# lh3/miniasm

Measured on NVIDIA H100. Metric: paf_overlaps_per_sec_ingest_to_gfa, higher is better.
Workload: dtype int64/uint32 (+3 float32 predicates)

## Files before the change

### miniasm_b200/csrc/asg_dev.cu

```cuda
#include "asg_dev.cuh"
#include <cub/cub.cuh>

int mab_verbose = 3;
thread_local int mab_mute = 0;
int mab_del_trans_count_inner = 0;
thread_local DelTransStats g_del_trans_stats;

__device__ __forceinline__ DArc ld_arc(const DArc *p)
{
	uint4 t = *reinterpret_cast<const uint4*>(p);
	DArc a;
	a.ul = (uint64_t)t.y << 32 | t.x; a.v = t.z; a.ol_del = t.w;
	return a;
}
__device__ __forceinline__ DArc ld_arc_nc(const DArc *p)
{
	uint4 t = __ldg(reinterpret_cast<const uint4*>(p));
	DArc a;
	a.ul = (uint64_t)t.y << 32 | t.x; a.v = t.z; a.ol_del = t.w;
	return a;
}

__device__ __forceinline__ uint4 ld_arc4(const DArc *p)
{
// ... 47 lines not shown
	{
		DArc a = ld_arc_nc(arc + i);
		if (flag && flag[i]) return false;
		if (a.ol_del & MAB_DEL_BIT) return false;
		uint32_t u = (uint32_t)(a.ul >> 32);
		return !((seq[u >> 1] | seq[a.v >> 1]) & MAB_DEL_BIT);
	}
};

__global__ void k_arc_count_dead(ArcKeep keep, uint32_t n, unsigned long long *n_dead)
{
	unsigned dead = 0;
	for (uint32_t i = blockIdx.x * blockDim.x + threadIdx.x; i < n; i += gridDim.x * blockDim.x) dead += !keep(i);
	dead = __reduce_add_sync(0xffffffffu, dead);
	if ((threadIdx.x & 31) == 0 && dead) atomicAdd(n_dead, (unsigned long long)dead);
}

void dg_arc_rm(MabDev &d, DGraph &g, const uint8_t *flag)
{
	if (g.n_arc == 0) return;
	cub::CountingInputIterator<uint32_t> cnt(0);
	ArcKeep keep{g.arc, g.seq, flag};
	if (!flag && g.n_arc > (1u << 20)) {
		d.zero_scal(SC_NSEL);
		MAB_LAUNCH(d, k_arc_count_dead, mab_grid(g.n_arc, 256), 256, 0, keep, g.n_arc, d.d_scal + SC_NSEL);
		if (d.get_scal(SC_NSEL) == 0) return;
	}
	cub::TransformInputIterator<bool, ArcKeep, cub::CountingInputIterator<uint32_t>> flags(cnt, keep);
	size_t tb = 0;
	unsigned long long *d_n = d.d_scal + SC_NSEL;
// ... 606 lines not shown
```

### miniasm_b200/csrc/asg_dev.cuh

```cuda
#pragma once
#include "mab_common.cuh"

struct DGraph {
	uint32_t n_seq = 0;
	uint32_t n_arc = 0;
	size_t   m_arc = 0;
	bool is_srt = false, is_symm = false, has_idx = false;
	uint32_t len_bits = 32;
	DArc *arc = nullptr;
	DArc *arc2 = nullptr;
	uint32_t *seq = nullptr;
	uint64_t *idx = nullptr;
};

void dg_reserve(MabDev &d, DGraph &g, size_t m_arc);
void dg_set_nseq(MabDev &d, DGraph &g, uint32_t n_seq);
void dg_free(MabDev &d, DGraph &g);

void dg_arc_rm(MabDev &d, DGraph &g, const uint8_t *flag);
void dg_arc_sort(MabDev &d, DGraph &g);
void dg_build_sorted(MabDev &d, DGraph &g, uint64_t *key, uint64_t *val, uint64_t *key2, uint64_t *val2, uint32_t n_in, uint32_t n_real, uint32_t lb, bool has_sentinel);
void dg_arc_index(MabDev &d, DGraph &g);
void dg_cleanup(MabDev &d, DGraph &g, const uint8_t *flag = nullptr);
uint32_t dg_del_multi(MabDev &d, DGraph &g);
uint32_t dg_del_asymm(MabDev &d, DGraph &g);
void dg_symm(MabDev &d, DGraph &g);
uint32_t dg_del_trans(MabDev &d, DGraph &g, uint32_t fuzz);
uint32_t dg_del_trans_flags(MabDev &d, DGraph &g, uint32_t fuzz, uint32_t own_lo, uint32_t own_hi, uint8_t **flag_out,
                            const DArc *const *peer = nullptr, const uint64_t *nidx = nullptr, const uint32_t *orig = nullptr, uint32_t world = 1);
uint32_t dg_del_short(MabDev &d, DGraph &g, float ratio);

struct DelTransStats { uint64_t n_arc_in, n_vtx, inner_iters, n_reduced, n_big; float kernel_ms; };
extern thread_local DelTransStats g_del_trans_stats;

// ... 5 lines not shown
```

### miniasm_b200/csrc/capi_fused.cu

```cuda
#include "../../include/miniasm_b200.h"
#include "capi_util.cuh"
#include "hit_dev.cuh"
#include "clean_dev.cuh"
#include "gfa_dev.cuh"
#include "dump_dev.cuh"
#include "ugseq_dev.cuh"
#include <pthread.h>
#include "ingest_dev.cuh"
#include "shard_comm.cuh"
#include <cub/cub.cuh>
#include <map>
#include <string>
#include <zlib.h>
#include <fcntl.h>
#include <unistd.h>
#include <sys/stat.h>

ma_ug_t *mab_ug_download(MabDev &d, DUnitigs &du);
extern "C" sdict_t *sd_from_packed(char *block, size_t block_size, uint32_t n, const uint32_t *len);

struct mab_ctx {
	MabDev dev;
	char *d_text = nullptr;
	size_t text_len = 0, text_cap = 0;
// ... 793 lines not shown
	dg_arc_rm(d, loc, nullptr);
	DGraph &g = c->sg;
	uint32_t n_keep = 0;
	DArc *keep = nullptr;
	uint64_t n_red_all = 0, tot = 0;
	std::vector<uint64_t> cnt = sc_allgather_u64(d, sc, loc.n_arc);
	for (int r = 0; r < G; ++r) tot += cnt[r];
	if (tot >= (1ull << 31)) { fprintf(stderr, "[E::miniasm_b200] more than 2^31 arcs in the graph\n"); exit(73); }
	c->stats.n_arc_sg = tot;
	if (MAB_V(1)) fprintf(stderr, "[M::%s] read %d arcs\n", "ma_sg_gen", (int)tot);
	std::vector<void*> peer_any;
	const bool p2p = sc_peer_ptrs(d, sc, loc.arc, peer_any);
	std::vector<const DArc*> peer_ptr((size_t)G, nullptr);
	for (int r = 0; r < G; ++r) peer_ptr[r] = (const DArc*)peer_any[r];
	if (p2p) {
		dg_arc_index(d, loc);
		uint64_t *nidx = mab_alloc<uint64_t>(d, (size_t)n * 2);
		if (n) MAB_CUDA(cudaMemcpyAsync(nidx, loc.idx, (size_t)n * 16, cudaMemcpyDeviceToDevice, d.stream));
		sc_allreduce(d, sc, nidx, (size_t)n * 2, ncclUint64, ncclSum);
		const DArc **d_peer = (const DArc**)d.alloc(sizeof(void*) * (size_t)G);
		MAB_CUDA(cudaMemcpyAsync(d_peer, peer_ptr.data(), sizeof(void*) * (size_t)G, cudaMemcpyHostToDevice, d.stream));
		uint8_t *flag = nullptr;
		uint32_t n_red = dg_del_trans_flags(d, loc, (uint32_t)opt->gap_fuzz, 0, 0xffffffffu, &flag, d_peer, nidx, c->orig_id, (uint32_t)G);
		c->stats.ms_del_trans_kernel = g_del_trans_stats.kernel_ms, c->stats.trans_inner = g_del_trans_stats.inner_iters;
		std::vector<uint64_t> reds = sc_allgather_u64(d, sc, n_red);
		for (int r = 0; r < G; ++r) n_red_all += reds[r];
		keep = mab_alloc<DArc>(d, loc.n_arc);
		if (loc.n_arc) {
			uint8_t *nf = mab_alloc<uint8_t>(d, loc.n_arc);
			MAB_LAUNCH(d, k_not_flag, mab_grid(loc.n_arc, 256), 256, 0, flag, loc.n_arc, nf);
			size_t tb = 0;
// ... 68 lines not shown
```

### miniasm_b200/csrc/hit_dev.cu

```cuda
#include "hit_dev.cuh"
#include "hit2arc.cuh"
#include <cub/cub.cuh>
#include <functional>

extern "C" int ma_verbose;
extern "C" const char *sys_timestamp(void);
#define ma_verbose_dev (mab_mute ? 0 : ma_verbose)

thread_local MabCountHook mab_count_hook = nullptr;
thread_local void *mab_count_hook_ctx = nullptr;
static inline void sum_ranks(unsigned long long *v, int n) { if (mab_count_hook) mab_count_hook(mab_count_hook_ctx, v, n); }

__device__ __forceinline__ DHit ld_hit(const DHit *p)
{
	const uint4 *q = reinterpret_cast<const uint4*>(p);
	uint4 a = __ldg(q), b = __ldg(q + 1);
	DHit h;
	h.qns = (uint64_t)a.y << 32 | a.x; h.qe = a.z; h.tn = a.w;
	h.ts = b.x; h.te = b.y; h.ml_rev = b.z; h.bl_del = b.w;
	return h;
}
__device__ __forceinline__ DHit ld_hit_rw(const DHit *p)
{
	const uint4 *q = reinterpret_cast<const uint4*>(p);
// ... 385 lines not shown
{
	drop_bounds(d, h);
	const uint32_t n_seq = h.n_seq;
	if (h.n == 0 || n_seq == 0) return;
	if (h.n >= (1ull << 32)) { fprintf(stderr, "[E::miniasm_b200] more than 2^32 hits on one GPU\n"); exit(73); }
	uint32_t *cnt = mab_alloc<uint32_t>(d, (size_t)n_seq + 1), *first = mab_alloc<uint32_t>(d, (size_t)n_seq + 1);
	MAB_CUDA(cudaMemsetAsync(cnt, 0, ((size_t)n_seq + 1) * 4, d.stream));
	MAB_LAUNCH(d, k_bucket_count, mab_grid(h.n, 256), 256, 0, h.a, h.n, cnt);
	dh_bucket_first(d, cnt, n_seq, first);
	MAB_CUDA(cudaMemsetAsync(cnt, 0, (size_t)n_seq * 4, d.stream));
	MAB_LAUNCH(d, k_bucket_fill, mab_grid(h.n, 256), 256, 0, h.a, h.n, first, cnt, h.a2);
	dh_sort_buckets(d, h, first);
	d.free(cnt); d.free(first);
}

__global__ void k_group_bounds(const DHit *a, size_t n, uint32_t *g32)
{
	for (size_t i = blockIdx.x * (size_t)blockDim.x + threadIdx.x; i < n; i += (size_t)gridDim.x * blockDim.x) {
		uint32_t q = (uint32_t)(a[i].qns >> 32);
		if (i == 0 || (uint32_t)(a[i - 1].qns >> 32) != q) g32[2 * (size_t)q + 1] = (uint32_t)i;
		if (i == n - 1 || (uint32_t)(a[i + 1].qns >> 32) != q) g32[2 * (size_t)q] = (uint32_t)(i + 1);
	}
}

__global__ void k_sub_keys(const DHit *a, size_t n, const uint64_t *__restrict__ grp, float min_iden, uint32_t clip, uint64_t *key)
{
	for (size_t i = blockIdx.x * (size_t)blockDim.x + threadIdx.x; i < n; i += (size_t)gridDim.x * blockDim.x) {
		DHit h = ld_hit(a + i);
		uint32_t qid = (uint32_t)(h.qns >> 32);
		int ml = (int)(h.ml_rev & 0x7fffffffu), bl = (int)(h.bl_del & 0x7fffffffu);
		bool skip = i >= (uint32_t)grp[qid] || h.tn == qid || (float)ml < __fmul_rn((float)bl, min_iden);
		uint32_t qs = (uint32_t)h.qns + clip, qe = h.qe - clip;
		uint64_t base = (uint64_t)qid << 33;
		if (!skip && qe > qs) {
			key[2 * i] = base | (uint32_t)(qs << 1);
			key[2 * i + 1] = base | (uint32_t)(qe << 1 | 1);
		} else {
// ... 339 lines not shown
	}
	d.free(huge);
}

uint64_t dh_sub(MabDev &d, const DHits &h, int min_dp, float min_iden, int end_clip, DSub *sub_out)
{
	const uint32_t n_seq = h.n_seq;
	unsigned long long n_remained = 0;
	if (n_seq) MAB_CUDA(cudaMemsetAsync(sub_out, 0, (size_t)n_seq * sizeof(DSub), d.stream));
	if (h.n && n_seq) {
		if (h.n >= (1ull << 31)) { fprintf(stderr, "[E::miniasm_b200] more than 2^31 hits on one GPU\n"); exit(73); }
		uint64_t *grp = h.grp;
		if (!grp) {
			grp = mab_alloc<uint64_t>(d, n_seq);
			MAB_CUDA(cudaMemsetAsync(grp, 0, (size_t)n_seq * 8, d.stream));
			MAB_LAUNCH(d, k_group_bounds, mab_grid(h.n, 256), 256, 0, h.a, h.n, (uint32_t*)grp);
		}
		uint32_t *big = mab_alloc<uint32_t>(d, n_seq);
		MAB_CUDA(cudaMemsetAsync(d.d_scal, 0, 8 * sizeof(unsigned long long), d.stream));
		unsigned grid = (n_seq + SUBW_WARPS - 1) / SUBW_WARPS;
		if (grid > MAB_SMS * 32u) grid = MAB_SMS * 32u;
		MAB_LAUNCH(d, k_sub_warp, grid, SUBW_WARPS * 32, 0, h.a, grp, n_seq, min_dp, min_iden, (uint32_t)end_clip, sub_out, big, d.d_scal);
		uint32_t n_big = (uint32_t)d.get_scal(SC_BIG);
		if (n_big) sub_big_reads(d, h, grp, big, n_big, min_dp, min_iden, end_clip, sub_out);
		n_remained = d.get_scal(SC_COUNT);
		if (grp != h.grp) d.free(grp);
		d.free(big);
	}
	sum_ranks(&n_remained, 1);
	if (ma_verbose_dev >= 3)
		fprintf(stderr, "[M::%s::%s] %ld query sequences remain after sub\n", "ma_hit_sub", sys_timestamp(), (long)n_remained);
// ... 327 lines not shown
	const int lane = threadIdx.x & 31;
	for (uint32_t r = (blockIdx.x * blockDim.x + threadIdx.x) >> 5; r < n_seq; r += (gridDim.x * blockDim.x) >> 5) {
		const int32_t m = map[r];
		if (m < 0) continue;
		const uint64_t g = grp[r];
		const uint32_t end = (uint32_t)g, first = (uint32_t)(g >> 32);
		unsigned c = 0;
		if (end) for (uint32_t i = first + lane; i < end; i += 32) c += map[tn[i]] >= 0;
		c = __reduce_add_sync(0xffffffffu, c);
		if (lane == 0) cnt[m] = c;
	}
}

__global__ void __launch_bounds__(256)
k_sel_final_copy(const DHit *__restrict__ a, const uint64_t *__restrict__ grp, const int32_t *__restrict__ map, uint32_t n_seq,
                 const uint32_t *__restrict__ off, const uint32_t *__restrict__ n_new, DHit *__restrict__ out, unsigned long long *scal)
{
	const int lane = threadIdx.x & 31;
	const unsigned lt = (1u << lane) - 1u;
	if (blockIdx.x == 0 && threadIdx.x == 0) { const uint32_t nn = *n_new; scal[SCS_NSEQ] = nn, scal[SCS_NHITS] = off[nn]; }
	for (uint32_t r = (blockIdx.x * blockDim.x + threadIdx.x) >> 5; r < n_seq; r += (gridDim.x * blockDim.x) >> 5) {
		const int32_t m = map[r];
		if (m < 0) continue;
		const uint64_t g = grp[r];
		const uint32_t end = (uint32_t)g, first = (uint32_t)(g >> 32);
		if (end == 0) continue;
		uint32_t o = off[m];
		for (uint32_t c = first; c < end; c += 32) {
			const uint32_t i = c + lane;
			DHit h;
			int32_t tn = -1;
			if (i < end) { h = ld_hit(a + i); tn = map[h.tn]; }
			const unsigned km = __ballot_sync(0xffffffffu, tn >= 0);
			if (tn >= 0) {
				h.qns = (uint64_t)(uint32_t)m << 32 | (uint32_t)h.qns, h.tn = (uint32_t)tn;
				st_hit(out + o + __popc(km & lt), h);
			}
			o += __popc(km);
// ... 11 lines not shown
{
	size_t tb = 0;
	cub::DeviceScan::ExclusiveSum(nullptr, tb, in, out, (int64_t)n, d.stream);
	void *tmp = d.tmp(tb);
	cub::DeviceScan::ExclusiveSum(tmp, tb, in, out, (int64_t)n, d.stream);
	++d.n_lib;
}

size_t dh_select(MabDev &d, DHits &h, DSub *sub, const SelectParams &o, int32_t *map_out, float *cov, const SelectHooks &hk)
{
	const uint32_t n_seq = h.n_seq;
	if (h.n >= (1ull << 31)) { fprintf(stderr, "[E::miniasm_b200] more than 2^31 hits on one GPU\n"); exit(73); }
	if (!h.grp) {
		h.grp = mab_alloc<uint64_t>(d, n_seq);
		MAB_CUDA(cudaMemsetAsync(h.grp, 0, (size_t)n_seq * 8, d.stream));
		if (h.n) MAB_LAUNCH(d, k_group_bounds, mab_grid(h.n, 256), 256, 0, h.a, h.n, (uint32_t*)h.grp);
	}
	dh_sub(d, h, o.min_dp, o.min_iden, 0, sub);
	if (hk.sub_done) hk.sub_done(sub);
	d.trace("select:sub1");

	const int clip = o.min_span / 2;
	DSub *sub2 = mab_alloc<DSub>(d, n_seq);
	uint32_t *big = mab_alloc<uint32_t>(d, n_seq);
	MAB_CUDA(cudaMemsetAsync(sub2, 0, (size_t)n_seq * sizeof(DSub), d.stream));
	d.zero_scal(0, SCS_NHITS + 1);
	MAB_LAUNCH(d, k_sel_cut_flt_sub, warp_grid(n_seq, SUBW_WARPS), SUBW_WARPS * 32, 0, h.a, h.grp, n_seq, sub, o.min_span, o.flt_max_hang, o.flt_min_ovlp,
	           o.min_dp, o.min_iden, (uint32_t)clip, sub2, big, d.d_scal);
	const uint32_t n_big = (uint32_t)d.get_scal(SC_BIG);
	{
		unsigned long long gv[4] = { d.h_scal[SCS_DP], d.h_scal[SCS_LEN], d.h_scal[SCS_CUT], d.h_scal[SCS_FLT] };
// ... 18 lines not shown

	uint8_t *used = mab_alloc<uint8_t>(d, n_seq);
	uint32_t *tn = reinterpret_cast<uint32_t*>(h.a2);
	MAB_CUDA(cudaMemsetAsync(used, 0, n_seq, d.stream));
	MAB_LAUNCH(d, k_sel_cut_cont, warp_grid(n_seq, 8), 256, 0, h.a, h.grp, n_seq, sub2, sub, o.min_span, o.cont, used, tn, d.d_scal + SCS_CUT2);
	if (hk.flags_done) hk.flags_done(sub, used, n_seq);

	uint32_t *keep = mab_alloc<uint32_t>(d, (size_t)n_seq + 1), *excl = mab_alloc<uint32_t>(d, (size_t)n_seq + 1);
	uint32_t *cnt = mab_alloc<uint32_t>(d, (size_t)n_seq + 1), *off = mab_alloc<uint32_t>(d, (size_t)n_seq + 1);
	MAB_CUDA(cudaMemsetAsync(keep + n_seq, 0, 4, d.stream));
	MAB_LAUNCH(d, k_cont_keep, mab_grid(n_seq, 256), 256, 0, n_seq, sub, used, nullptr, keep);
	exclusive_sum(d, keep, excl, (size_t)n_seq + 1);
	MAB_LAUNCH(d, k_cont_map, mab_grid(n_seq, 256), 256, 0, n_seq, keep, excl, map_out, sub, sub2);
	MAB_LAUNCH(d, k_sel_final_count, warp_grid(n_seq, 8), 256, 0, h.grp, tn, map_out, n_seq, cnt);
	exclusive_sum(d, cnt, off, (size_t)n_seq + 1);
	MAB_LAUNCH(d, k_sel_final_copy, warp_grid(n_seq, 8), 256, 0, h.a, h.grp, map_out, n_seq, off, excl + n_seq, h.a2, d.d_scal);
	const uint32_t n_new = (uint32_t)d.get_scal(SCS_NSEQ);
	const size_t n_hits = (size_t)d.h_scal[SCS_NHITS];
	const unsigned long long n_cut2 = d.h_scal[SCS_CUT2];
	if (n_new) MAB_CUDA(cudaMemcpyAsync(sub, sub2, (size_t)n_new * sizeof(DSub), cudaMemcpyDeviceToDevice, d.stream));
	d.free(sub2); d.free(used); d.free(keep); d.free(excl); d.free(cnt); d.free(off);
	DHit *t = h.a; h.a = h.a2; h.a2 = t;
	h.n = n_hits, h.n_seq = n_new;
	drop_bounds(d, h);
	d.trace("select:cut2+contained");

	unsigned long long gv[2] = { n_cut2, (unsigned long long)h.n };
	sum_ranks(gv, 2);
	if (ma_verbose_dev >= 3) {
		fprintf(stderr, "[M::%s::%s] %ld hits remain after cut\n", "ma_hit_cut", sys_timestamp(), (long)gv[0]);
		fprintf(stderr, "[M::%s::%s] %d sequences and %ld hits remain after containment removal\n", "ma_hit_contained", sys_timestamp(), n_new, (long)gv[1]);
	}
	return h.n;
}

__global__ void k_seq_set(uint32_t n_seq, const uint32_t *len, const uint8_t *del, uint32_t *seq, unsigned *max_len)
{
	unsigned mx = 0;
	for (uint32_t i = blockIdx.x * blockDim.x + threadIdx.x; i < n_seq; i += gridDim.x * blockDim.x) {
// ... 17 lines not shown
		bool emit = false;
		if (r >= 0) {
			if (qn == h.tn) {
				if ((uint32_t)h.qns == h.ts && h.qe == h.te && (h.ml_rev >> 31)) atomicOr(&seq[qn], MAB_DEL_BIT);
			} else emit = true;
		} else if (r == MAB_HT_QCONT) atomicOr(&seq[qn], MAB_DEL_BIT);
		key[i] = emit ? ((t.ul >> 32) << lb | (uint32_t)t.ul) : sentinel;
		val[i] = (uint64_t)t.ol_del << 32 | t.v;
		cnt += emit;
	}
	cnt = __reduce_add_sync(0xffffffffu, cnt);
	if ((threadIdx.x & 31) == 0 && cnt) atomicAdd(n_emit, (unsigned long long)cnt);
}

constexpr int SGW_WARPS = 8, SGW_HITS = 256, SGW_IDX_BITS = 9;
constexpr int SGC_HITS = 8192;

__global__ void k_sg_classify(const DHit *a, size_t n, uint32_t *seq, HitArcParams p, uint8_t *emit_flag, uint32_t *g32, unsigned long long *scal)
{
	unsigned cnt = 0;
	bool bad = false;
	for (size_t i = blockIdx.x * (size_t)blockDim.x + threadIdx.x; i < n; i += (size_t)gridDim.x * blockDim.x) {
		DHit h = ld_hit(a + i);
		const uint32_t qn = (uint32_t)(h.qns >> 32);
		DArc t;
		t.ul = 0, t.v = 0, t.ol_del = 0;
		const int r = mab_hit2arc(h, (int)(seq[qn] & 0x7fffffffu), (int)(seq[h.tn] & 0x7fffffffu), p.max_hang, p.int_frac, p.min_ovlp, &t);
		bool emit = false;
		if (r >= 0) {
			if (qn == h.tn) {
				if ((uint32_t)h.qns == h.ts && h.qe == h.te && (h.ml_rev >> 31)) atomicOr(&seq[qn], MAB_DEL_BIT);
			} else emit = true;
		} else if (r == MAB_HT_QCONT) atomicOr(&seq[qn], MAB_DEL_BIT);
		emit_flag[i] = emit;
		cnt += emit;
		const uint32_t prev = i ? (uint32_t)(a[i - 1].qns >> 32) : 0;
		if (i == 0 || prev != qn) g32[2 * (size_t)qn + 1] = (uint32_t)i;
		if (i == n - 1 || (uint32_t)(a[i + 1].qns >> 32) != qn) g32[2 * (size_t)qn] = (uint32_t)(i + 1);
		if (i && prev > qn) bad = true;
	}
	cnt = __reduce_add_sync(0xffffffffu, cnt);
	if ((threadIdx.x & 31) == 0 && cnt) atomicAdd(scal + SC_COUNT, (unsigned long long)cnt);
	if (bad) scal[SC_AUX2] = 1ull;
}

struct U8ToU32 { __host__ __device__ __forceinline__ uint32_t operator()(uint8_t x) const { return x; } };

__global__ void __launch_bounds__(SGW_WARPS * 32)
k_sg_sort_warp(const DHit *__restrict__ a, const uint64_t *__restrict__ grp, const uint32_t *__restrict__ epos, const uint32_t *__restrict__ seq,
               uint32_t n_seq, HitArcParams p, uint32_t lb, DArc *__restrict__ out, uint32_t *big_list, unsigned long long *scal)
{
	__shared__ uint32_t s_key[SGW_WARPS][SGW_HITS], s_v[SGW_WARPS][SGW_HITS], s_ol[SGW_WARPS][SGW_HITS];
	const int warp = threadIdx.x >> 5, lane = threadIdx.x & 31;
	uint32_t *key = s_key[warp], *pv = s_v[warp], *pol = s_ol[warp];
	const uint32_t len_mask = (1u << lb) - 1u;
	for (uint32_t r = blockIdx.x * SGW_WARPS + warp; r < n_seq; r += gridDim.x * SGW_WARPS) {
		const uint64_t g = grp[r];
		const uint32_t end = (uint32_t)g, first = (uint32_t)(g >> 32);
		if (end == 0) continue;
		const uint32_t cnt = end - first;
		if (cnt > SGW_HITS) { if (lane == 0) big_list[atomicAdd(scal + SC_BIG, 1ull)] = r; continue; }
		const int ql = (int)(seq[r] & 0x7fffffffu);
		uint32_t n = 0;
		for (uint32_t c = 0; c < cnt; c += 32) {
			bool ok = false;
			DArc t;
			t.ul = 0, t.v = 0, t.ol_del = 0;
			if (c + lane < cnt) {
				const DHit h = ld_hit(a + first + c + lane);
				const int rr = mab_hit2arc(h, ql, (int)(seq[h.tn] & 0x7fffffffu), p.max_hang, p.int_frac, p.min_ovlp, &t);
				ok = rr >= 0 && h.tn != r;
			}
			const unsigned m = __ballot_sync(0xffffffffu, ok);
			if (ok) {
				const uint32_t k = n + __popc(m & ((1u << lane) - 1u));
				key[k] = ((((uint32_t)(t.ul >> 32) & 1u) << lb | (uint32_t)t.ul) << SGW_IDX_BITS) | k;
				pv[k] = t.v, pol[k] = t.ol_del;
			}
			n += __popc(m);
		}
		if (n == 0) continue;
		uint32_t np = 32; while (np < n) np <<= 1;
		__syncwarp();
		switch (np) {
			case 32: sub_sort_regs<1>(key, n, lane); break;
			case 64: sub_sort_regs<2>(key, n, lane); break;
			case 128: sub_sort_regs<4>(key, n, lane); break;
			default: sub_sort_regs<8>(key, n, lane); break;
		}
		__syncwarp();
		const uint32_t base = epos[first];
		for (uint32_t j = lane; j < n; j += 32) {
			const uint32_t k = key[j], src = k & ((1u << SGW_IDX_BITS) - 1u), kl = k >> SGW_IDX_BITS;
			*reinterpret_cast<uint4*>(out + base + j) = make_uint4(kl & len_mask, r << 1 | kl >> lb, pv[src], pol[src]);
		}
		__syncwarp();
	}
}

__global__ void __launch_bounds__(512)
k_sg_sort_cta(const DHit *__restrict__ a, const uint64_t *__restrict__ grp, const uint32_t *__restrict__ epos, const uint32_t *__restrict__ seq,
              const uint32_t *__restrict__ big_list, uint32_t n_big, HitArcParams p, DArc *__restrict__ out, unsigned long long *scal)
{
	extern __shared__ __align__(16) unsigned char sg_smem[];
	uint64_t *key = reinterpret_cast<uint64_t*>(sg_smem);
	uint32_t *pv = reinterpret_cast<uint32_t*>(key + SGC_HITS), *pol = pv + SGC_HITS;
	__shared__ uint32_t s_n;
	const uint32_t tid = threadIdx.x, nt = blockDim.x;
	for (uint32_t b = blockIdx.x; b < n_big; b += gridDim.x) {
		const uint32_t r = big_list[b];
		const uint64_t g = grp[r];
		const uint32_t first = (uint32_t)(g >> 32), cnt = (uint32_t)g - first;
		if (cnt > SGC_HITS) { if (tid == 0) atomicAdd(scal + SC_AUX, 1ull); continue; }
		if (tid == 0) s_n = 0;
		__syncthreads();
		const uint32_t base = epos[first];
		const int ql = (int)(seq[r] & 0x7fffffffu);
		for (uint32_t c = tid; c < cnt; c += nt) {
			const DHit h = ld_hit(a + first + c);
			DArc t;
			t.ul = 0, t.v = 0, t.ol_del = 0;
			const int rr = mab_hit2arc(h, ql, (int)(seq[h.tn] & 0x7fffffffu), p.max_hang, p.int_frac, p.min_ovlp, &t);
			if (rr >= 0 && h.tn != r) {
				const uint32_t k = epos[first + c] - base;
				key[k] = (uint64_t)((((uint32_t)(t.ul >> 32) & 1u) << 31) | (uint32_t)t.ul) << 32 | k;
				pv[k] = t.v, pol[k] = t.ol_del;
				atomicAdd(&s_n, 1u);
			}
		}
		__syncthreads();
		const uint32_t n = s_n;
		uint32_t np = 2; while (np < n) np <<= 1;
		for (uint32_t i = n + tid; i < np; i += nt) key[i] = ~0ull;
		__syncthreads();
		for (uint32_t k = 2, lk = 1; k <= np; k <<= 1, ++lk)
			for (uint32_t lj = lk; lj-- > 0;) {
				const uint32_t j = 1u << lj;
				for (uint32_t t = tid; t < np / 2; t += nt) {
					const uint32_t lo = ((t >> lj) << (lj + 1)) | (t & (j - 1)), hi = lo + j;
					const uint64_t x = key[lo], y = key[hi];
					const bool asc = (lo & k) == 0;
					if ((x > y) == asc) key[lo] = y, key[hi] = x;
				}
				__syncthreads();
			}
		for (uint32_t j = tid; j < n; j += nt) {
			const uint64_t k = key[j];
			const uint32_t src = (uint32_t)k, kl = (uint32_t)(k >> 32);
			*reinterpret_cast<uint4*>(out + base + j) = make_uint4(kl & 0x7fffffffu, r << 1 | kl >> 31, pv[src], pol[src]);
		}
		__syncthreads();
	}
}

static bool sg_emit_segmented(MabDev &d, const DHits &h, const HitArcParams &p, uint32_t lb, DGraph &g)
{
	const size_t n = h.n;
	const uint32_t n_seq = h.n_seq;
	if (lb + 1 + SGW_IDX_BITS > 32 || n >= (1ull << 31)) return false;
	uint8_t *ef = mab_alloc<uint8_t>(d, n);
	uint32_t *epos = mab_alloc<uint32_t>(d, n), *big = mab_alloc<uint32_t>(d, n_seq);
	uint64_t *grp = mab_alloc<uint64_t>(d, n_seq);
	MAB_CUDA(cudaMemsetAsync(grp, 0, (size_t)n_seq * 8, d.stream));
	d.zero_scal(SC_COUNT, 5);
	MAB_LAUNCH(d, k_sg_classify, mab_grid(n, 256), 256, 0, h.a, n, g.seq, p, ef, (uint32_t*)grp, d.d_scal);
	const uint32_t n_arc = (uint32_t)d.get_scal(SC_COUNT);
	bool ok = d.h_scal[SC_AUX2] == 0;
	if (ok) {
		cub::TransformInputIterator<uint32_t, U8ToU32, const uint8_t*> in(ef, U8ToU32());
		size_t tb = 0;
		cub::DeviceScan::ExclusiveSum(nullptr, tb, in, epos, (int64_t)n, d.stream);
		void *tmp = d.tmp(tb);
		cub::DeviceScan::ExclusiveSum(tmp, tb, in, epos, (int64_t)n, d.stream);
		++d.n_lib;
		dg_reserve(d, g, n_arc ? n_arc : 1);
		unsigned grid = (n_seq + SGW_WARPS - 1) / SGW_WARPS;
		if (grid > MAB_SMS * 32u) grid = MAB_SMS * 32u;
		MAB_LAUNCH(d, k_sg_sort_warp, grid, SGW_WARPS * 32, 0, h.a, grp, epos, g.seq, n_seq, p, lb, g.arc, big, d.d_scal);
		const uint32_t n_big = (uint32_t)d.get_scal(SC_BIG);
		if (n_big) {
				const size_t smem = (size_t)SGC_HITS * 16;
			MAB_CUDA(cudaFuncSetAttribute(k_sg_sort_cta, cudaFuncAttributeMaxDynamicSharedMemorySize, (int)smem));
			MAB_LAUNCH(d, k_sg_sort_cta, n_big < MAB_SMS ? n_big : MAB_SMS, 512, smem, h.a, grp, epos, g.seq, big, n_big, p, g.arc, d.d_scal);
			if (d.get_scal(SC_AUX) != 0) ok = false;
		}
	}
	d.free(ef); d.free(epos); d.free(big); d.free(grp);
	if (ok) g.len_bits = lb, g.n_arc = n_arc, g.is_srt = true, g.has_idx = false;
	return ok;
}

void dh_sg_gen(MabDev &d, const DHits &h, const uint32_t *len, const uint8_t *del, const HitArcParams &p, DGraph &g)
{
	dh_sg_emit(d, h, len, del, p, g);
	dg_cleanup(d, g);
	if (MAB_V(1)) fprintf(stderr, "[M::%s] read %d arcs\n", "ma_sg_gen", g.n_arc);
}

void dh_sg_emit(MabDev &d, const DHits &h, const uint32_t *len, const uint8_t *del, const HitArcParams &p, DGraph &g)
{
	const uint32_t n_seq = h.n_seq;
	dg_set_nseq(d, g, n_seq);
	g.n_arc = 0, g.is_srt = false, g.is_symm = false, g.has_idx = false;
	d.zero_scal(SC_AUX);
	d.zero_scal(SC_COUNT);
	unsigned *d_max = (unsigned*)(d.d_scal + SC_AUX);
	if (n_seq) MAB_LAUNCH(d, k_seq_set, mab_grid(n_seq, 256), 256, 0, n_seq, len, del, g.seq, d_max);
	const unsigned mx = (unsigned)(d.get_scal(SC_AUX) & 0xffffffffu);
	const uint32_t lb = bits_for(mx);
	if (h.n) {
		if (h.n >= (1ull << 31)) { fprintf(stderr, "[E::miniasm_b200] more than 2^31 arcs on one GPU\n"); exit(73); }
		static const bool seg_sort = !(getenv("MAB_SG_SEGSORT") && atoi(getenv("MAB_SG_SEGSORT")) == 0);
		if (seg_sort && sg_emit_segmented(d, h, p, lb, g)) return;
		if (seg_sort) d.zero_scal(SC_COUNT);
		const uint64_t sentinel = 1ull << (lb + bits_for((uint64_t)n_seq * 2 - 1));
		uint64_t *ka = mab_alloc<uint64_t>(d, h.n), *kb = mab_alloc<uint64_t>(d, h.n), *va = mab_alloc<uint64_t>(d, h.n), *vb = mab_alloc<uint64_t>(d, h.n);
		MAB_LAUNCH(d, k_sg_arcs, mab_grid(h.n, 256), 256, 0, h.a, h.n, g.seq, p, lb, sentinel, ka, va, d.d_scal + SC_COUNT);
		const uint32_t n_arc = (uint32_t)d.get_scal(SC_COUNT);
		dg_build_sorted(d, g, ka, va, kb, vb, (uint32_t)h.n, n_arc, lb, true);
		d.free(ka); d.free(kb); d.free(va); d.free(vb);
	} else { dg_reserve(d, g, 1); g.is_srt = true; }
}
```

### miniasm_b200/csrc/hit_dev.cuh

```cuda
#pragma once
#include "mab_common.cuh"
#include "asg_dev.cuh"
#include <functional>

typedef void (*MabCountHook)(void *ctx, unsigned long long *v, int n);
extern thread_local MabCountHook mab_count_hook;
extern thread_local void *mab_count_hook_ctx;

struct DHits {
	DHit *a = nullptr, *a2 = nullptr;
	size_t n = 0, m = 0;
	uint32_t n_seq = 0;
	uint64_t *grp = nullptr;
};

struct HitArcParams { int max_hang; float int_frac; int min_ovlp; };

void dh_reserve(MabDev &d, DHits &h, size_t m);
void dh_free(MabDev &d, DHits &h);

void dh_sort(MabDev &d, DHits &h);
void dh_bucket_first(MabDev &d, const uint32_t *cnt, uint32_t n_seq, uint32_t *first);
void dh_sort_buckets(MabDev &d, DHits &h, const uint32_t *first);

// ... 1 lines not shown

size_t dh_cut(MabDev &d, DHits &h, const DSub *reg, int min_span);

size_t dh_flt(MabDev &d, DHits &h, const DSub *sub, int max_hang, int min_ovlp, float *cov);

void dh_sub_merge(MabDev &d, uint32_t n_sub, DSub *a, const DSub *b);

size_t dh_contained(MabDev &d, DHits &h, DSub *sub, const uint8_t *seq_del, const HitArcParams &p, int32_t *map_out);
struct SelectParams { int min_dp; float min_iden; int min_span; int flt_max_hang, flt_min_ovlp; HitArcParams cont; };
struct SelectHooks {
	std::function<void()> step3;
	std::function<void(DSub*)> sub_done;
	std::function<void(DSub*, uint8_t*, uint32_t)> flags_done;
};
size_t dh_select(MabDev &d, DHits &h, DSub *sub, const SelectParams &o, int32_t *map_out, float *cov, const SelectHooks &hk);
void dh_sg_emit(MabDev &d, const DHits &h, const uint32_t *len, const uint8_t *del, const HitArcParams &p, DGraph &g);

void dh_sg_gen(MabDev &d, const DHits &h, const uint32_t *len, const uint8_t *del, const HitArcParams &p, DGraph &g);
```

Baseline: 1.451 billion.

## Fuse arc classification, scan and per-read sort into single-pass kernel

Replaces the classify, device-scan and warp-sort pipeline for string-graph arc emission with one kernel that computes arcs per read, sorts them in shared memory, and gets output offsets through a decoupled look-back tile prefix. The kernel also writes the arc index directly and counts deleted reads, so cleanup and reindexing can be skipped when nothing was deleted. Group bounds are now reused from the selection step instead of being recomputed. The intent is to cut passes over the hit array, temporary buffers and host syncs. The cost is a more complex kernel with tile-ordering dependencies and atomics on the seq flags.

Result: faster. 1.546 billion (median of 6 runs) (+6.6%).

```diff
diff --git a/miniasm_b200/csrc/asg_dev.cu b/miniasm_b200/csrc/asg_dev.cu
--- a/miniasm_b200/csrc/asg_dev.cu
+++ b/miniasm_b200/csrc/asg_dev.cu
@@ -85,6 +85,22 @@
 	for (uint32_t i = blockIdx.x * blockDim.x + threadIdx.x; i < n; i += gridDim.x * blockDim.x) dead += !keep(i);
 	dead = __reduce_add_sync(0xffffffffu, dead);
 	if ((threadIdx.x & 31) == 0 && dead) atomicAdd(n_dead, (unsigned long long)dead);
+}
+
+__global__ void k_seq_count_del(const uint32_t *seq, uint32_t n, unsigned long long *n_del)
+{
+	unsigned c = 0;
+	for (uint32_t i = blockIdx.x * blockDim.x + threadIdx.x; i < n; i += gridDim.x * blockDim.x) c += seq[i] >> 31;
+	c = __reduce_add_sync(0xffffffffu, c);
+	if ((threadIdx.x & 31) == 0 && c) atomicAdd(n_del, (unsigned long long)c);
+}
+
+uint32_t dg_n_del_seq(MabDev &d, const DGraph &g)
+{
+	if (g.n_seq == 0) return 0;
+	d.zero_scal(SC_NSEL);
+	MAB_LAUNCH(d, k_seq_count_del, mab_grid(g.n_seq, 256), 256, 0, g.seq, g.n_seq, d.d_scal + SC_NSEL);
+	return (uint32_t)d.get_scal(SC_NSEL);
 }
 
 void dg_arc_rm(MabDev &d, DGraph &g, const uint8_t *flag)
diff --git a/miniasm_b200/csrc/asg_dev.cuh b/miniasm_b200/csrc/asg_dev.cuh
--- a/miniasm_b200/csrc/asg_dev.cuh
+++ b/miniasm_b200/csrc/asg_dev.cuh
@@ -18,6 +18,7 @@
 void dg_free(MabDev &d, DGraph &g);
 
 void dg_arc_rm(MabDev &d, DGraph &g, const uint8_t *flag);
+uint32_t dg_n_del_seq(MabDev &d, const DGraph &g);
 void dg_arc_sort(MabDev &d, DGraph &g);
 void dg_build_sorted(MabDev &d, DGraph &g, uint64_t *key, uint64_t *val, uint64_t *key2, uint64_t *val2, uint32_t n_in, uint32_t n_real, uint32_t lb, bool has_sentinel);
 void dg_arc_index(MabDev &d, DGraph &g);
diff --git a/miniasm_b200/csrc/capi_fused.cu b/miniasm_b200/csrc/capi_fused.cu
--- a/miniasm_b200/csrc/capi_fused.cu
+++ b/miniasm_b200/csrc/capi_fused.cu
@@ -831,7 +831,7 @@
 	std::vector<const DArc*> peer_ptr((size_t)G, nullptr);
 	for (int r = 0; r < G; ++r) peer_ptr[r] = (const DArc*)peer_any[r];
 	if (p2p) {
-		dg_arc_index(d, loc);
+		if (!loc.has_idx) dg_arc_index(d, loc);
 		uint64_t *nidx = mab_alloc<uint64_t>(d, (size_t)n * 2);
 		if (n) MAB_CUDA(cudaMemcpyAsync(nidx, loc.idx, (size_t)n * 16, cudaMemcpyDeviceToDevice, d.stream));
 		sc_allreduce(d, sc, nidx, (size_t)n * 2, ncclUint64, ncclSum);
diff --git a/miniasm_b200/csrc/hit_dev.cu b/miniasm_b200/csrc/hit_dev.cu
--- a/miniasm_b200/csrc/hit_dev.cu
+++ b/miniasm_b200/csrc/hit_dev.cu
@@ -423,13 +423,16 @@
 	d.free(cnt); d.free(first);
 }
 
-__global__ void k_group_bounds(const DHit *a, size_t n, uint32_t *g32)
-{
+__global__ void k_group_bounds(const DHit *a, size_t n, uint32_t *g32, unsigned long long *unsorted)
+{
+	bool bad = false;
 	for (size_t i = blockIdx.x * (size_t)blockDim.x + threadIdx.x; i < n; i += (size_t)gridDim.x * blockDim.x) {
-		uint32_t q = (uint32_t)(a[i].qns >> 32);
-		if (i == 0 || (uint32_t)(a[i - 1].qns >> 32) != q) g32[2 * (size_t)q + 1] = (uint32_t)i;
+		uint32_t q = (uint32_t)(a[i].qns >> 32), prev = i ? (uint32_t)(a[i - 1].qns >> 32) : 0;
+		if (i == 0 || prev != q) g32[2 * (size_t)q + 1] = (uint32_t)i;
 		if (i == n - 1 || (uint32_t)(a[i + 1].qns >> 32) != q) g32[2 * (size_t)q] = (uint32_t)(i + 1);
-	}
+		bad |= i && prev > q;
+	}
+	if (bad && unsorted) *unsorted = 1ull;
 }
 
 __global__ void k_sub_keys(const DHit *a, size_t n, const uint64_t *__restrict__ grp, float min_iden, uint32_t clip, uint64_t *key)
@@ -799,7 +802,7 @@
 		if (!grp) {
 			grp = mab_alloc<uint64_t>(d, n_seq);
 			MAB_CUDA(cudaMemsetAsync(grp, 0, (size_t)n_seq * 8, d.stream));
-			MAB_LAUNCH(d, k_group_bounds, mab_grid(h.n, 256), 256, 0, h.a, h.n, (uint32_t*)grp);
+			MAB_LAUNCH(d, k_group_bounds, mab_grid(h.n, 256), 256, 0, h.a, h.n, (uint32_t*)grp, nullptr);
 		}
 		uint32_t *big = mab_alloc<uint32_t>(d, n_seq);
 		MAB_CUDA(cudaMemsetAsync(d.d_scal, 0, 8 * sizeof(unsigned long long), d.stream));
@@ -1157,7 +1160,8 @@
 
 __global__ void __launch_bounds__(256)
 k_sel_final_copy(const DHit *__restrict__ a, const uint64_t *__restrict__ grp, const int32_t *__restrict__ map, uint32_t n_seq,
-                 const uint32_t *__restrict__ off, const uint32_t *__restrict__ n_new, DHit *__restrict__ out, unsigned long long *scal)
+                 const uint32_t *__restrict__ off, const uint32_t *__restrict__ n_new, DHit *__restrict__ out, uint64_t *__restrict__ grp_out,
+                 unsigned long long *scal)
 {
 	const int lane = threadIdx.x & 31;
 	const unsigned lt = (1u << lane) - 1u;
@@ -1165,6 +1169,7 @@
 	for (uint32_t r = (blockIdx.x * blockDim.x + threadIdx.x) >> 5; r < n_seq; r += (gridDim.x * blockDim.x) >> 5) {
 		const int32_t m = map[r];
 		if (m < 0) continue;
+		if (lane == 0) { const uint32_t s = off[m], e = off[m + 1]; grp_out[m] = e > s ? (uint64_t)s << 32 | e : 0; }
 		const uint64_t g = grp[r];
 		const uint32_t end = (uint32_t)g, first = (uint32_t)(g >> 32);
 		if (end == 0) continue;
@@ -1206,7 +1211,7 @@
 	if (!h.grp) {
 		h.grp = mab_alloc<uint64_t>(d, n_seq);
 		MAB_CUDA(cudaMemsetAsync(h.grp, 0, (size_t)n_seq * 8, d.stream));
-		if (h.n) MAB_LAUNCH(d, k_group_bounds, mab_grid(h.n, 256), 256, 0, h.a, h.n, (uint32_t*)h.grp);
+		if (h.n) MAB_LAUNCH(d, k_group_bounds, mab_grid(h.n, 256), 256, 0, h.a, h.n, (uint32_t*)h.grp, nullptr);
 	}
 	dh_sub(d, h, o.min_dp, o.min_iden, 0, sub);
 	if (hk.sub_done) hk.sub_done(sub);
@@ -1255,7 +1260,8 @@
 	MAB_LAUNCH(d, k_cont_map, mab_grid(n_seq, 256), 256, 0, n_seq, keep, excl, map_out, sub, sub2);
 	MAB_LAUNCH(d, k_sel_final_count, warp_grid(n_seq, 8), 256, 0, h.grp, tn, map_out, n_seq, cnt);
 	exclusive_sum(d, cnt, off, (size_t)n_seq + 1);
-	MAB_LAUNCH(d, k_sel_final_copy, warp_grid(n_seq, 8), 256, 0, h.a, h.grp, map_out, n_seq, off, excl + n_seq, h.a2, d.d_scal);
+	uint64_t *grp_new = mab_alloc<uint64_t>(d, n_seq);
+	MAB_LAUNCH(d, k_sel_final_copy, warp_grid(n_seq, 8), 256, 0, h.a, h.grp, map_out, n_seq, off, excl + n_seq, h.a2, grp_new, d.d_scal);
 	const uint32_t n_new = (uint32_t)d.get_scal(SCS_NSEQ);
 	const size_t n_hits = (size_t)d.h_scal[SCS_NHITS];
 	const unsigned long long n_cut2 = d.h_scal[SCS_CUT2];
@@ -1263,7 +1269,8 @@
 	d.free(sub2); d.free(used); d.free(keep); d.free(excl); d.free(cnt); d.free(off);
 	DHit *t = h.a; h.a = h.a2; h.a2 = t;
 	h.n = n_hits, h.n_seq = n_new;
-	drop_bounds(d, h);
+	d.free(h.grp);
+	h.grp = grp_new;
 	d.trace("select:cut2+contained");
 
 	unsigned long long gv[2] = { n_cut2, (unsigned long long)h.n };
@@ -1311,72 +1318,71 @@
 }
 
 constexpr int SGW_WARPS = 8, SGW_HITS = 256, SGW_IDX_BITS = 9;
-constexpr int SGC_HITS = 8192;
-
-__global__ void k_sg_classify(const DHit *a, size_t n, uint32_t *seq, HitArcParams p, uint8_t *emit_flag, uint32_t *g32, unsigned long long *scal)
-{
-	unsigned cnt = 0;
-	bool bad = false;
-	for (size_t i = blockIdx.x * (size_t)blockDim.x + threadIdx.x; i < n; i += (size_t)gridDim.x * blockDim.x) {
-		DHit h = ld_hit(a + i);
-		const uint32_t qn = (uint32_t)(h.qns >> 32);
-		DArc t;
-		t.ul = 0, t.v = 0, t.ol_del = 0;
-		const int r = mab_hit2arc(h, (int)(seq[qn] & 0x7fffffffu), (int)(seq[h.tn] & 0x7fffffffu), p.max_hang, p.int_frac, p.min_ovlp, &t);
-		bool emit = false;
-		if (r >= 0) {
-			if (qn == h.tn) {
-				if ((uint32_t)h.qns == h.ts && h.qe == h.te && (h.ml_rev >> 31)) atomicOr(&seq[qn], MAB_DEL_BIT);
-			} else emit = true;
-		} else if (r == MAB_HT_QCONT) atomicOr(&seq[qn], MAB_DEL_BIT);
-		emit_flag[i] = emit;
-		cnt += emit;
-		const uint32_t prev = i ? (uint32_t)(a[i - 1].qns >> 32) : 0;
-		if (i == 0 || prev != qn) g32[2 * (size_t)qn + 1] = (uint32_t)i;
-		if (i == n - 1 || (uint32_t)(a[i + 1].qns >> 32) != qn) g32[2 * (size_t)qn] = (uint32_t)(i + 1);
-		if (i && prev > qn) bad = true;
-	}
-	cnt = __reduce_add_sync(0xffffffffu, cnt);
-	if ((threadIdx.x & 31) == 0 && cnt) atomicAdd(scal + SC_COUNT, (unsigned long long)cnt);
-	if (bad) scal[SC_AUX2] = 1ull;
-}
-
-struct U8ToU32 { __host__ __device__ __forceinline__ uint32_t operator()(uint8_t x) const { return x; } };
+constexpr int SGC_HITS = 8192, SGC_THREADS = 512;
+
+typedef cub::ScanTileState<uint32_t> ArcTileState;
+typedef cub::TilePrefixCallbackOp<uint32_t, ::cuda::std::plus<uint32_t>, ArcTileState> ArcPrefixOp;
+
+__global__ void k_arc_tiles_init(ArcTileState ts, int n_tile) { ts.InitializeStatus(n_tile); }
+
+__global__ void k_grp_max(const uint64_t *grp, uint32_t n, unsigned long long *mx)
+{
+	unsigned m = 0;
+	for (uint32_t i = blockIdx.x * blockDim.x + threadIdx.x; i < n; i += gridDim.x * blockDim.x) {
+		const uint64_t g = grp[i];
+		const unsigned c = (uint32_t)g ? (uint32_t)g - (uint32_t)(g >> 32) : 0;
+		m = c > m ? c : m;
+	}
+	m = __reduce_max_sync(0xffffffffu, m);
+	if ((threadIdx.x & 31) == 0 && m) atomicMax(mx, (unsigned long long)m);
+}
 
 __global__ void __launch_bounds__(SGW_WARPS * 32)
-k_sg_sort_warp(const DHit *__restrict__ a, const uint64_t *__restrict__ grp, const uint32_t *__restrict__ epos, const uint32_t *__restrict__ seq,
-               uint32_t n_seq, HitArcParams p, uint32_t lb, DArc *__restrict__ out, uint32_t *big_list, unsigned long long *scal)
+k_sg_onepass(const DHit *__restrict__ a, const uint64_t *__restrict__ grp, uint32_t *seq, uint32_t n_seq, HitArcParams p, uint32_t lb,
+             unsigned long long *tile_ctr, ArcTileState tstate, DArc *__restrict__ out, uint64_t *__restrict__ idx, uint2 *__restrict__ big_list,
+             unsigned long long *scal)
 {
 	__shared__ uint32_t s_key[SGW_WARPS][SGW_HITS], s_v[SGW_WARPS][SGW_HITS], s_ol[SGW_WARPS][SGW_HITS];
+	__shared__ typename ArcPrefixOp::TempStorage s_pref;
+	__shared__ uint32_t s_n[SGW_WARPS], s_tile, s_base;
 	const int warp = threadIdx.x >> 5, lane = threadIdx.x & 31;
+	const unsigned lt = (1u << lane) - 1u;
 	uint32_t *key = s_key[warp], *pv = s_v[warp], *pol = s_ol[warp];
 	const uint32_t len_mask = (1u << lb) - 1u;
-	for (uint32_t r = blockIdx.x * SGW_WARPS + warp; r < n_seq; r += gridDim.x * SGW_WARPS) {
+	if (threadIdx.x == 0) s_tile = (uint32_t)atomicAdd(tile_ctr, 1ull);
+	__syncthreads();
+	const uint32_t t = s_tile, r = t * SGW_WARPS + warp;
+	uint32_t first = 0, cnt = 0, n = 0, n0 = 0;
+	int ql = 0;
+	if (r < n_seq) {
 		const uint64_t g = grp[r];
-		const uint32_t end = (uint32_t)g, first = (uint32_t)(g >> 32);
-		if (end == 0) continue;
-		const uint32_t cnt = end - first;
-		if (cnt > SGW_HITS) { if (lane == 0) big_list[atomicAdd(scal + SC_BIG, 1ull)] = r; continue; }
-		const int ql = (int)(seq[r] & 0x7fffffffu);
-		uint32_t n = 0;
-		for (uint32_t c = 0; c < cnt; c += 32) {
-			bool ok = false;
-			DArc t;
-			t.ul = 0, t.v = 0, t.ol_del = 0;
-			if (c + lane < cnt) {
-				const DHit h = ld_hit(a + first + c + lane);
-				const int rr = mab_hit2arc(h, ql, (int)(seq[h.tn] & 0x7fffffffu), p.max_hang, p.int_frac, p.min_ovlp, &t);
-				ok = rr >= 0 && h.tn != r;
-			}
-			const unsigned m = __ballot_sync(0xffffffffu, ok);
-			if (ok) {
-				const uint32_t k = n + __popc(m & ((1u << lane) - 1u));
-				key[k] = ((((uint32_t)(t.ul >> 32) & 1u) << lb | (uint32_t)t.ul) << SGW_IDX_BITS) | k;
-				pv[k] = t.v, pol[k] = t.ol_del;
-			}
-			n += __popc(m);
-		}
-		if (n == 0) continue;
+		if ((uint32_t)g) first = (uint32_t)(g >> 32), cnt = (uint32_t)g - first;
+		ql = (int)(seq[r] & 0x7fffffffu);
+	}
+	const bool big = cnt > SGW_HITS;
+	for (uint32_t c = 0; c < cnt; c += 32) {
+		bool ok = false;
+		DArc e;
+		e.ul = 0, e.v = 0, e.ol_del = 0;
+		if (c + lane < cnt) {
+			const DHit h = ld_hit(a + first + c + lane);
+			const int rr = mab_hit2arc(h, ql, (int)(seq[h.tn] & 0x7fffffffu), p.max_hang, p.int_frac, p.min_ovlp, &e);
+			if (rr >= 0) {
+				if (h.tn == r) {
+					if ((uint32_t)h.qns == h.ts && h.qe == h.te && (h.ml_rev >> 31)) atomicOr(&seq[r], MAB_DEL_BIT);
+				} else ok = true;
+			} else if (rr == MAB_HT_QCONT) atomicOr(&seq[r], MAB_DEL_BIT);
+		}
+		const uint32_t dir = (uint32_t)(e.ul >> 32) & 1u;
+		const unsigned m = __ballot_sync(0xffffffffu, ok), m0 = __ballot_sync(0xffffffffu, ok && dir == 0);
+		if (ok && !big) {
+			const uint32_t k = n + __popc(m & lt);
+			key[k] = ((dir << lb | (uint32_t)e.ul) << SGW_IDX_BITS) | k;
+			pv[k] = e.v, pol[k] = e.ol_del;
+		}
+		n += __popc(m), n0 += __popc(m0);
+	}
+	if (n && !big) {
 		uint32_t np = 32; while (np < n) np <<= 1;
 		__syncwarp();
 		switch (np) {
@@ -1386,47 +1392,76 @@
 			default: sub_sort_regs<8>(key, n, lane); break;
 		}
 		__syncwarp();
-		const uint32_t base = epos[first];
-		for (uint32_t j = lane; j < n; j += 32) {
-			const uint32_t k = key[j], src = k & ((1u << SGW_IDX_BITS) - 1u), kl = k >> SGW_IDX_BITS;
-			*reinterpret_cast<uint4*>(out + base + j) = make_uint4(kl & len_mask, r << 1 | kl >> lb, pv[src], pol[src]);
-		}
-		__syncwarp();
-	}
-}
-
-__global__ void __launch_bounds__(512)
-k_sg_sort_cta(const DHit *__restrict__ a, const uint64_t *__restrict__ grp, const uint32_t *__restrict__ epos, const uint32_t *__restrict__ seq,
-              const uint32_t *__restrict__ big_list, uint32_t n_big, HitArcParams p, DArc *__restrict__ out, unsigned long long *scal)
-{
+	}
+	if (lane == 0) {
+		s_n[warp] = n;
+		if (r < n_seq && (atomicOr(&seq[r], 0u) & MAB_DEL_BIT)) atomicAdd(scal + SC_NSEL, 1ull);
+	}
+	__syncthreads();
+	if (warp == 0) {
+		const uint32_t agg = __reduce_add_sync(0xffffffffu, lane < SGW_WARPS ? s_n[lane] : 0u);
+		if (t == 0) {
+			if (lane == 0) tstate.SetInclusive(0, agg), s_base = 0;
+		} else {
+			ArcPrefixOp op(tstate, s_pref, ::cuda::std::plus<uint32_t>(), (int)t);
+			const uint32_t ex = op(agg);
+			if (lane == 0) s_base = ex;
+		}
+		if (lane == 0 && agg) atomicAdd(scal + SC_COUNT, (unsigned long long)agg);
+	}
+	__syncthreads();
+	if (r >= n_seq) return;
+	uint32_t base = s_base;
+	for (int w = 0; w < warp; ++w) base += s_n[w];
+	if (lane == 0) {
+		idx[2 * (size_t)r] = n0 ? (uint64_t)base << 32 | n0 : 0;
+		idx[2 * (size_t)r + 1] = n > n0 ? (uint64_t)(base + n0) << 32 | (n - n0) : 0;
+		if (big && n) big_list[atomicAdd(scal + SC_BIG, 1ull)] = make_uint2(r, base);
+	}
+	if (big) return;
+	for (uint32_t j = lane; j < n; j += 32) {
+		const uint32_t k = key[j], src = k & ((1u << SGW_IDX_BITS) - 1u), kl = k >> SGW_IDX_BITS;
+		*reinterpret_cast<uint4*>(out + base + j) = make_uint4(kl & len_mask, r << 1 | kl >> lb, pv[src], pol[src]);
+	}
+}
+
+__global__ void __launch_bounds__(SGC_THREADS)
+k_sg_sort_cta(const DHit *__restrict__ a, const uint64_t *__restrict__ grp, const uint32_t *__restrict__ seq,
+              const uint2 *__restrict__ big_list, uint32_t n_big, HitArcParams p, DArc *__restrict__ out)
+{
+	typedef cub::BlockScan<uint32_t, SGC_THREADS> BS;
 	extern __shared__ __align__(16) unsigned char sg_smem[];
 	uint64_t *key = reinterpret_cast<uint64_t*>(sg_smem);
 	uint32_t *pv = reinterpret_cast<uint32_t*>(key + SGC_HITS), *pol = pv + SGC_HITS;
-	__shared__ uint32_t s_n;
+	__shared__ typename BS::TempStorage s_scan;
 	const uint32_t tid = threadIdx.x, nt = blockDim.x;
 	for (uint32_t b = blockIdx.x; b < n_big; b += gridDim.x) {
-		const uint32_t r = big_list[b];
+		const uint2 rb = big_list[b];
+		const uint32_t r = rb.x, base = rb.y;
 		const uint64_t g = grp[r];
 		const uint32_t first = (uint32_t)(g >> 32), cnt = (uint32_t)g - first;
-		if (cnt > SGC_HITS) { if (tid == 0) atomicAdd(scal + SC_AUX, 1ull); continue; }
-		if (tid == 0) s_n = 0;
-		__syncthreads();
-		const uint32_t base = epos[first];
 		const int ql = (int)(seq[r] & 0x7fffffffu);
-		for (uint32_t c = tid; c < cnt; c += nt) {
-			const DHit h = ld_hit(a + first + c);
-			DArc t;
-			t.ul = 0, t.v = 0, t.ol_del = 0;
-			const int rr = mab_hit2arc(h, ql, (int)(seq[h.tn] & 0x7fffffffu), p.max_hang, p.int_frac, p.min_ovlp, &t);
-			if (rr >= 0 && h.tn != r) {
-				const uint32_t k = epos[first + c] - base;
-				key[k] = (uint64_t)((((uint32_t)(t.ul >> 32) & 1u) << 31) | (uint32_t)t.ul) << 32 | k;
-				pv[k] = t.v, pol[k] = t.ol_del;
-				atomicAdd(&s_n, 1u);
+		uint32_t n = 0;
+		for (uint32_t c0 = 0; c0 < cnt; c0 += nt) {
+			const uint32_t c = c0 + tid;
+			bool ok = false;
+			DArc e;
+			e.ul = 0, e.v = 0, e.ol_del = 0;
+			if (c < cnt) {
+				const DHit h = ld_hit(a + first + c);
+				const int rr = mab_hit2arc(h, ql, (int)(seq[h.tn] & 0x7fffffffu), p.max_hang, p.int_frac, p.min_ovlp, &e);
+				ok = rr >= 0 && h.tn != r;
 			}
-		}
-		__syncthreads();
-		const uint32_t n = s_n;
+			uint32_t k, tot;
+			BS(s_scan).ExclusiveSum((uint32_t)ok, k, tot);
+			if (ok) {
+				k += n;
+				key[k] = (uint64_t)((((uint32_t)(e.ul >> 32) & 1u) << 31) | (uint32_t)e.ul) << 32 | k;
+				pv[k] = e.v, pol[k] = e.ol_del;
+			}
+			n += tot;
+			__syncthreads();
+		}
 		uint32_t np = 2; while (np < n) np <<= 1;
 		for (uint32_t i = n + tid; i < np; i += nt) key[i] = ~0ull;
 		__syncthreads();
@@ -1450,51 +1485,59 @@
 	}
 }
 
-static bool sg_emit_segmented(MabDev &d, const DHits &h, const HitArcParams &p, uint32_t lb, DGraph &g)
+static bool sg_emit_segmented(MabDev &d, const DHits &h, const HitArcParams &p, uint32_t lb, DGraph &g, uint32_t *n_del)
 {
 	const size_t n = h.n;
 	const uint32_t n_seq = h.n_seq;
-	if (lb + 1 + SGW_IDX_BITS > 32 || n >= (1ull << 31)) return false;
-	uint8_t *ef = mab_alloc<uint8_t>(d, n);
-	uint32_t *epos = mab_alloc<uint32_t>(d, n), *big = mab_alloc<uint32_t>(d, n_seq);
-	uint64_t *grp = mab_alloc<uint64_t>(d, n_seq);
-	MAB_CUDA(cudaMemsetAsync(grp, 0, (size_t)n_seq * 8, d.stream));
+	if (lb + 1 + SGW_IDX_BITS > 32 || n >= (1ull << 31) || n_seq == 0) return false;
 	d.zero_scal(SC_COUNT, 5);
-	MAB_LAUNCH(d, k_sg_classify, mab_grid(n, 256), 256, 0, h.a, n, g.seq, p, ef, (uint32_t*)grp, d.d_scal);
-	const uint32_t n_arc = (uint32_t)d.get_scal(SC_COUNT);
-	bool ok = d.h_scal[SC_AUX2] == 0;
+	d.zero_scal(SC_NSEL);
+	d.zero_scal(SC_TMP0);
+	const uint64_t *grp = h.grp;
+	uint64_t *own = nullptr;
+	if (!grp) {
+		own = mab_alloc<uint64_t>(d, n_seq);
+		MAB_CUDA(cudaMemsetAsync(own, 0, (size_t)n_seq * 8, d.stream));
+		MAB_LAUNCH(d, k_group_bounds, mab_grid(n, 256), 256, 0, h.a, n, (uint32_t*)own, d.d_scal + SC_AUX2);
+		grp = own;
+	}
+	MAB_LAUNCH(d, k_grp_max, mab_grid(n_seq, 256), 256, 0, grp, n_seq, d.d_scal + SC_AUX);
+	const bool ok = d.get_scal(SC_AUX) <= (unsigned long long)SGC_HITS && d.h_scal[SC_AUX2] == 0;
 	if (ok) {
-		cub::TransformInputIterator<uint32_t, U8ToU32, const uint8_t*> in(ef, U8ToU32());
-		size_t tb = 0;
-		cub::DeviceScan::ExclusiveSum(nullptr, tb, in, epos, (int64_t)n, d.stream);
-		void *tmp = d.tmp(tb);
-		cub::DeviceScan::ExclusiveSum(tmp, tb, in, epos, (int64_t)n, d.stream);
-		++d.n_lib;
-		dg_reserve(d, g, n_arc ? n_arc : 1);
-		unsigned grid = (n_seq + SGW_WARPS - 1) / SGW_WARPS;
-		if (grid > MAB_SMS * 32u) grid = MAB_SMS * 32u;
-		MAB_LAUNCH(d, k_sg_sort_warp, grid, SGW_WARPS * 32, 0, h.a, grp, epos, g.seq, n_seq, p, lb, g.arc, big, d.d_scal);
-		const uint32_t n_big = (uint32_t)d.get_scal(SC_BIG);
+		dg_reserve(d, g, n);
+		const int n_tile = (int)((n_seq + SGW_WARPS - 1) / SGW_WARPS);
+		size_t ts_bytes = 0;
+		MAB_CUDA(ArcTileState::AllocationSize(n_tile, ts_bytes));
+		void *ts_mem = d.alloc(ts_bytes);
+		ArcTileState ts;
+		MAB_CUDA(ts.Init(n_tile, ts_mem, ts_bytes));
+		MAB_LAUNCH(d, k_arc_tiles_init, mab_grid((size_t)n_tile, 256, 1u << 30), 256, 0, ts, n_tile);
+		uint2 *big = mab_alloc<uint2>(d, n_seq);
+		MAB_LAUNCH(d, k_sg_onepass, n_tile, SGW_WARPS * 32, 0, h.a, grp, g.seq, n_seq, p, lb, d.d_scal + SC_TMP0, ts, g.arc, g.idx, big, d.d_scal);
+		g.n_arc = (uint32_t)d.get_scal(SC_COUNT);
+		*n_del = (uint32_t)d.h_scal[SC_NSEL];
+		const uint32_t n_big = (uint32_t)d.h_scal[SC_BIG];
 		if (n_big) {
-				const size_t smem = (size_t)SGC_HITS * 16;
+			const size_t smem = (size_t)SGC_HITS * 16;
 			MAB_CUDA(cudaFuncSetAttribute(k_sg_sort_cta, cudaFuncAttributeMaxDynamicSharedMemorySize, (int)smem));
-			MAB_LAUNCH(d, k_sg_sort_cta, n_big < MAB_SMS ? n_big : MAB_SMS, 512, smem, h.a, grp, epos, g.seq, big, n_big, p, g.arc, d.d_scal);
-			if (d.get_scal(SC_AUX) != 0) ok = false;
-		}
-	}
-	d.free(ef); d.free(epos); d.free(big); d.free(grp);
-	if (ok) g.len_bits = lb, g.n_arc = n_arc, g.is_srt = true, g.has_idx = false;
+			MAB_LAUNCH(d, k_sg_sort_cta, n_big < MAB_SMS ? n_big : MAB_SMS, SGC_THREADS, smem, h.a, grp, g.seq, big, n_big, p, g.arc);
+		}
+		d.free(ts_mem); d.free(big);
+		g.len_bits = lb, g.is_srt = true, g.has_idx = true;
+	}
+	d.free(own);
 	return ok;
 }
 
 void dh_sg_gen(MabDev &d, const DHits &h, const uint32_t *len, const uint8_t *del, const HitArcParams &p, DGraph &g)
 {
-	dh_sg_emit(d, h, len, del, p, g);
-	dg_cleanup(d, g);
+	const int64_t n_del = dh_sg_emit(d, h, len, del, p, g);
+	if ((n_del < 0 ? dg_n_del_seq(d, g) : (uint32_t)n_del) != 0) dg_cleanup(d, g);
+	else if (!g.has_idx) dg_arc_index(d, g);
 	if (MAB_V(1)) fprintf(stderr, "[M::%s] read %d arcs\n", "ma_sg_gen", g.n_arc);
 }
 
-void dh_sg_emit(MabDev &d, const DHits &h, const uint32_t *len, const uint8_t *del, const HitArcParams &p, DGraph &g)
+int64_t dh_sg_emit(MabDev &d, const DHits &h, const uint32_t *len, const uint8_t *del, const HitArcParams &p, DGraph &g)
 {
 	const uint32_t n_seq = h.n_seq;
 	dg_set_nseq(d, g, n_seq);
@@ -1508,8 +1551,9 @@
 	if (h.n) {
 		if (h.n >= (1ull << 31)) { fprintf(stderr, "[E::miniasm_b200] more than 2^31 arcs on one GPU\n"); exit(73); }
 		static const bool seg_sort = !(getenv("MAB_SG_SEGSORT") && atoi(getenv("MAB_SG_SEGSORT")) == 0);
-		if (seg_sort && sg_emit_segmented(d, h, p, lb, g)) return;
-		if (seg_sort) d.zero_scal(SC_COUNT);
+		uint32_t n_del = 0;
+		if (seg_sort && sg_emit_segmented(d, h, p, lb, g, &n_del)) return n_del;
+		d.zero_scal(SC_COUNT);
 		const uint64_t sentinel = 1ull << (lb + bits_for((uint64_t)n_seq * 2 - 1));
 		uint64_t *ka = mab_alloc<uint64_t>(d, h.n), *kb = mab_alloc<uint64_t>(d, h.n), *va = mab_alloc<uint64_t>(d, h.n), *vb = mab_alloc<uint64_t>(d, h.n);
 		MAB_LAUNCH(d, k_sg_arcs, mab_grid(h.n, 256), 256, 0, h.a, h.n, g.seq, p, lb, sentinel, ka, va, d.d_scal + SC_COUNT);
@@ -1517,4 +1561,5 @@
 		dg_build_sorted(d, g, ka, va, kb, vb, (uint32_t)h.n, n_arc, lb, true);
 		d.free(ka); d.free(kb); d.free(va); d.free(vb);
 	} else { dg_reserve(d, g, 1); g.is_srt = true; }
-}
+	return -1;
+}
diff --git a/miniasm_b200/csrc/hit_dev.cuh b/miniasm_b200/csrc/hit_dev.cuh
--- a/miniasm_b200/csrc/hit_dev.cuh
+++ b/miniasm_b200/csrc/hit_dev.cuh
@@ -39,6 +39,6 @@
 	std::function<void(DSub*, uint8_t*, uint32_t)> flags_done;
 };
 size_t dh_select(MabDev &d, DHits &h, DSub *sub, const SelectParams &o, int32_t *map_out, float *cov, const SelectHooks &hk);
-void dh_sg_emit(MabDev &d, const DHits &h, const uint32_t *len, const uint8_t *del, const HitArcParams &p, DGraph &g);
+int64_t dh_sg_emit(MabDev &d, const DHits &h, const uint32_t *len, const uint8_t *del, const HitArcParams &p, DGraph &g);
 
 void dh_sg_gen(MabDev &d, const DHits &h, const uint32_t *len, const uint8_t *del, const HitArcParams &p, DGraph &g);
```
